# python-microscopy/ch-shrinkwrap

Measured on AMD Instinct MI355X. Metric: vertex-updates/s (force+CG step) + achieved HBM GB/s, 1M pts/200k verts, higher is better.
Workload: dtype f32; 1 GPU; BASELINE configs[2]: two-lobe vesicle (smooth union of two R=300 nm spheres), 1000000 localizations sigma=10 nm, 198812 vertices / 397620 faces, lams=[10], blocks of 5 iterations, fixed topology; localizations_per_gpu=1000000, vertices_per_gpu=198812, faces_per_gpu=397620, block=5, mode=single, parallelism=single GPU

## Files before the change

### ch_shrinkwrap_amd/build.py

```python
import glob
import os
import subprocess

HERE = os.path.dirname(os.path.abspath(__file__))
LIB = os.path.join(HERE, 'libnanowrap_hip.so')


def _csrc(name):
    return os.path.join(HERE, 'csrc', name)


def _include(name):
    return os.path.join(os.path.dirname(HERE), 'include', name)


HIPCC_FLAGS = ['-O3', '--offload-arch=gfx950', '-fPIC', '-shared', '-ffp-contract=off', '-munsafe-fp-atomics',
               '-fvisibility=hidden', '-Wall', '-Wno-unused-function']
_BASE = ['-O3', '--offload-arch=gfx950', '-fPIC', '-fvisibility=hidden']
_QUERY = _BASE + ['-ffp-contract=off', '-Wall', '-Wno-unused-function']
_BQ_H = [_csrc('nw_bq.h'), _csrc('nw_bq_core.h')]
_BQ = _BQ_H + [_csrc('nw_device.h')]

OBJ_MAIN, OBJ_HOLEPUNCH, OBJ_SURGERY, OBJ_BQ = _csrc('nanowrap.o'), _csrc('nw_holepunch.o'), _csrc('nw_surgery.o'), _csrc('nw_bq.o')
OBJ_ISOSURFACE = _csrc('nw_isosurface.o')
# ... 7 lines not shown
OBJ_PROXIMITY = _csrc('nw_proximity.o')
UNITS = [
    (_csrc('nanowrap.hip'), OBJ_MAIN, sorted(set(glob.glob(_csrc('*.h'))) - set(_BQ_H)) + [_include('nanowrap.h')],
     [f for f in HIPCC_FLAGS if f != '-shared']),
    (_csrc('nw_sort.hip'), _csrc('nw_sort.o'), [], _BASE + ['-Wno-unused-value']),
    (_csrc('nw_remesh_dev.hip'), _csrc('nw_remesh_dev.o'), [_include('nanowrap.h'), _csrc('nw_remesh_plan.h')],
     _BASE + ['-ffp-contract=off', '-Wall', '-Wno-unused-value', '-Wno-unused-function']),
    (_csrc('nw_holepunch.hip'), OBJ_HOLEPUNCH, [_include('nw_holepunch.h')] + _BQ_H, _QUERY),
    (_csrc('nw_surgery.hip'), OBJ_SURGERY, [_include('nw_surgery.h')] + _BQ, _QUERY),
    (_csrc('nw_isosurface.hip'), OBJ_ISOSURFACE, [_include('nw_isosurface.h')] + _BQ_H, _QUERY),
    (_csrc('nw_evaluation.hip'), OBJ_EVALUATION, [_include('nw_evaluation.h'), _csrc('nw_evaluation_core.h')] + _BQ_H, _QUERY),
    (_csrc('nw_simulation.hip'), OBJ_SIMULATION, [_include('nw_simulation.h')] + _BQ_H, _QUERY),
    (_csrc('nw_distance.hip'), OBJ_DISTANCE, [_include('nw_distance.h'), _csrc('nw_distance_core.h')] + _BQ_H, _QUERY),
    (_csrc('nw_neighbours.hip'), OBJ_NEIGHBOURS, [_include('nw_neighbours.h'), _csrc('nw_neighbours_core.h')] + _BQ_H, _QUERY),
    (_csrc('nw_intersections.hip'), OBJ_INTERSECTIONS, [_include('nw_intersections.h'), _csrc('nw_intersections_core.h')] + _BQ_H, _QUERY),
    (_csrc('nw_rays.hip'), OBJ_RAYS, [_include('nw_rays.h'), _csrc('nw_rays_core.h'), _csrc('nw_intersections_core.h')] + _BQ_H, _QUERY),
    (_csrc('nw_volume.hip'), OBJ_VOLUME, [_include('nw_volume.h'), _csrc('nw_volume_core.h'), _csrc('nw_distance_core.h')] + _BQ_H, _QUERY),
    (_csrc('nw_proximity.hip'), OBJ_PROXIMITY, [_include('nw_proximity.h'), _csrc('nw_proximity_core.h'), _csrc('nw_distance_core.h'),
                                                _csrc('nw_intersections_core.h')] + _BQ_H, _QUERY),
    (_csrc('nw_bq.hip'), OBJ_BQ, _BQ, _QUERY),
]
DEPS = sorted(set(d for src, _, extra, _ in UNITS for d in [src] + extra))


def needs_build():
    if not os.path.exists(LIB):
        return True
    t = os.path.getmtime(LIB)
    return any(os.path.getmtime(d) > t for d in DEPS)


def build_hip_library(force=False, verbose=False):
    if not force and not needs_build():
        return LIB
    hipcc = os.environ.get('HIPCC', '/opt/rocm/bin/hipcc')

    def run(cmd):
        if verbose:
            print(' '.join(cmd))
        subprocess.check_call(cmd)

    for src, obj, extra, flags in UNITS:
        if force or not os.path.exists(obj) or os.path.getmtime(obj) < max(os.path.getmtime(d) for d in [src] + extra):
            run([hipcc] + flags + ['-c', '-o', obj, src])
    check_kernel_budgets(verbose=verbose)
    run([hipcc, '--offload-arch=gfx950', '-fPIC', '-shared', '-o', LIB] + [obj for _, obj, _, _ in UNITS])
    return LIB


LLVM_BIN = os.environ.get('NW_LLVM_BIN', '/opt/rocm/lib/llvm/bin')
KERNEL_BUDGETS = {
    'k_nn_wave<false>':               (80, 10 * 1024),
    'k_attract':                      (72, 20 * 1024),
    'k_face_centroids':               (64, 8 * 1024),
    'k_centroid_scatter':             (64, 0),
    'k_scan_final':                   (64, 1024),
    'k_prior_ring':                   (128, 1024),
    'k_prior_directions':             (96, 1024),
    'k_subspace_point_sums':          (128, 1024),
    'k_solve_update':                 (128, 1024),
    'k_hp_empty_faces':               (64, 0),
    'k_hp_pair':                      (64, 8 * 1024),
    'k_hp_prism':                     (176, 0),
    'k_hp_cand_geom':                 (32, 0),
    'k_hp_pair_final':                (16, 0),
    'k_ws_init':                      (16, 0),
    'k_ws_hook':                      (32, 0),
    'k_ws_compress':                  (16, 0),
    'k_ws_number':                    (16, 0),
    'k_ws_stats':                     (64, 0),
    'k_ws_bbox_init':                 (16, 0),
    'k_ws_active':                    (16, 0),
    'k_ws_winding':                   (176, 0),
    'k_ws_lengths':                   (16, 0),
    'k_ws_hist':                      (16, 2048),
    'k_ws_pick':                      (32, 0),
    'k_ws_flag':                      (16, 0),
    'k_iso_count':                    (16, 16 * 1024),
    'k_iso_widen':                    (16, 0),
    'k_iso_smooth':                   (16, 0),
    'k_iso_hist':                     (16, 1024),
    'k_iso_pattern':                  (32, 0),
    'k_iso_compact':                  (16, 0),
    'k_iso_cell_counts':              (16, 0),
    'k_iso_vertices':                 (64, 0),
    'k_iso_quads':                    (32, 0),
    'k_ev_face_setup':                (64, 0),
    'k_ev_node_test':                 (32, 0),
    'k_ev_emit':                      (32, 0),
    'k_ev_nearest':                   (64, 64),
    'k_ev_sum_final':                 (16, 64),
    'k_sim_eval':                     (64, 0),
    'k_sim_normals':                  (72, 0),
    'k_sim_cell_test':                (64, 0),
    'k_sim_cell_split':               (24, 0),
    'k_sim_leaf_test':                (64, 0),
    'k_sim_leaf_emit':                (32, 0),
    'k_sim_project':                  (72, 0),
    'k_sim_loc_error':                (32, 0),
    'k_sim_displace':                 (56, 0),
    'k_sim_background':               (16, 0),
    'k_sim_copy_hist':                (16, 1024),
    'k_sim_copy_equal':               (16, 0),
    'k_sim_copy_keep':                (16, 0),
    'k_sim_copy_emit':                (88, 0),
    'k_md_face_setup':                (64, 0),
    'k_md_rho_reduce':                (24, 64),
# ... 116 lines not shown
```

### ch_shrinkwrap_amd/csrc/nanowrap.hip

```cpp
#include <hip/hip_runtime.h>
#include <cstdio>
#include <cstdlib>
#include <cstring>
#include <cmath>
#include <string>
#include <vector>
#include <algorithm>
#include <chrono>
#include <thread>
#include <atomic>

#include "../../include/nanowrap.h"
#include "nw_kernels.h"
#include "nw_host_copy.h"

int nw_sort_pairs_u32(const unsigned *key_in, unsigned *key_out, const int *val_in, int *val_out, int n, int bits, hipStream_t stream);

static_assert(sizeof(NwIterLogDev) == sizeof(nw_iter_log), "device/host log record mismatch");
static_assert(SC_COUNT <= NW_N_SCALARS, "scalar slots");

#define NW_EXPORT extern "C" __attribute__((visibility("default")))

#include <dlfcn.h>
#include <rccl/rccl.h>
// ... 196 lines not shown
    void *pin_log = nullptr;
    int *pin_flag = nullptr;
    DevBuf<int> done_count;
    int done_expected = 0;
    bool done_launched = false;
    double block_us_ema = 0.0;
    uint64_t block_us_key = 0;
    std::chrono::steady_clock::time_point block_t0;
    int sliced_S = 0, sliced_base = 0;
    int64_t sliced_rows = 0;
    size_t pin_log_bytes = 0;
    void *pin = nullptr;
    size_t pin_bytes = 0;
    void *pin_base = nullptr;
    int pin_sel = 0;
    bool rows_async = false;
    NwHostPool *pool = nullptr;
    std::vector<hipEvent_t> wb_events;
    std::vector<unsigned char> valid_host;

    int profiling = 0;
    std::vector<hipEvent_t> events;
    size_t ev_used = 0;
    double stage_ms[ST_COUNT] = {0};
    int64_t stage_launches[ST_COUNT] = {0};
};

namespace {

int fail(nw_ctx *c, int code, const std::string &msg)
{
    if (c) c->err = msg;
    return code;
}

bool env_on(const char *name) { const char *e = getenv(name); return !(e && atoi(e) == 0); }
int verbose_level() { const char *e = getenv("NW_VERBOSE"); return e ? atoi(e) : 0; }

#define NW_HIP(call)                                                                                         \
    do {                                                                                                     \
        hipError_t e_ = (call);                                                                              \
        if (e_ != hipSuccess)                                                                                \
            return fail(ctx, NW_ERR_HIP, std::string(#call) + ": " + hipGetErrorString(e_));                \
    } while (0)

#define NW_TRY(expr)                                                                                         \
    do {                                                                                                     \
        int r_ = (expr);                                                                                     \
        if (r_ != NW_OK) return r_;                                                                          \
    } while (0)

inline int nblk(int64_t n, int b = NW_BLOCK) { return (int)((n + b - 1) / b); }

int scan_exclusive(nw_ctx *ctx, int *in, int n, int *out, bool zero_input = false, int *tile_sums = nullptr)
{
    const int nb = (n + NW_SCAN_TILE - 1) / NW_SCAN_TILE;
    const bool two_pass = nb <= 4096;
    if (tile_sums && two_pass) {
        hipLaunchKernelGGL(k_scan_final, dim3(nb), dim3(NW_BLOCK), 0, ctx->stream, in, n, tile_sums, out, zero_input ? 1 : 0, 1);
        NW_HIP(hipGetLastError());
        return NW_OK;
    }
    NW_HIP(ctx->scan_tmp.ensure((size_t)nb + 1));
    hipLaunchKernelGGL(k_scan_tile_sums, dim3(nb), dim3(NW_BLOCK), 0, ctx->stream, in, n, ctx->scan_tmp.p);
    if (!two_pass) hipLaunchKernelGGL(k_scan_bsums, dim3(1), dim3(1024), 0, ctx->stream, ctx->scan_tmp.p, nb);
    hipLaunchKernelGGL(k_scan_final, dim3(nb), dim3(NW_BLOCK), 0, ctx->stream, in, n, ctx->scan_tmp.p, out, zero_input ? 1 : 0, two_pass ? 1 : 0);
    NW_HIP(hipGetLastError());
    return NW_OK;
}

float dec_ord(int v)
{
    unsigned u = v >= 0 ? (unsigned)v : (0x80000000u - (unsigned)v);
    float f;
    memcpy(&f, &u, 4);
    return f;
}

int enc_ord(float f)
{
    f = f + 0.0f;
    unsigned u;
    memcpy(&u, &f, 4);
    return f >= 0 ? (int)u : (int)(0x80000000u - u);
}

int minmax3(nw_ctx *ctx, const float *xyz, int64_t n, float lo[3], float hi[3], bool *nonfinite)
{
    NW_HIP(ctx->mm.ensure(8));
    int init[8];
    for (int k = 0; k < 3; ++k) { init[k] = enc_ord(INFINITY); init[3 + k] = enc_ord(-INFINITY); }
    init[6] = 0; init[7] = 0;
    NW_HIP(hipMemcpyAsync(ctx->mm.p, init, sizeof(init), hipMemcpyHostToDevice, ctx->stream));
    const int blocks = (int)std::min<int64_t>(2048, (n + NW_BLOCK - 1) / NW_BLOCK);
    hipLaunchKernelGGL(k_minmax3, dim3(blocks), dim3(NW_BLOCK), 0, ctx->stream, xyz, n, ctx->mm.p, (int *)(ctx->mm.p + 6));
    NW_HIP(hipGetLastError());
    int out[8];
    NW_HIP(hipMemcpyAsync(out, ctx->mm.p, sizeof(out), hipMemcpyDeviceToHost, ctx->stream));
    NW_HIP(hipStreamSynchronize(ctx->stream));
    for (int k = 0; k < 3; ++k) { lo[k] = dec_ord(out[k]); hi[k] = dec_ord(out[3 + k]); }
    if (nonfinite) *nonfinite = out[6] != 0;
    return NW_OK;
}

double desired_cell(const nw_ctx *ctx, double mean_dist, double spacing)
{
    const double ratio = std::max((double)ctx->N, 1.0) / (2.5 * std::max((double)ctx->F, 1.0));
    const double sp = std::max(spacing, 1e-30);
    const double sr = ctx->sigma_eff > 0 ? std::min(std::max(ctx->sigma_eff / sp, 1.0), 16.0) : 4.0;
    double h = 2.9 * sp * std::pow(sr, 0.3) * std::pow(ratio, -0.11);
    const char *e = getenv("NW_CELL_FACTOR");
    if (e && atof(e) > 0) h *= atof(e);
    return std::max(h, 0.5 * mean_dist) * ctx->cell_tune;
}

int ensure_item_done(nw_ctx *ctx)
{
    const size_t want = (size_t)std::max(ctx->nitems, 1) + 256;
    if (!ctx->query_serial.p) {
// ... 993 lines not shown
    if (ctx->profiling) { ctx->ev_used = 0; g_marks.spans.clear(); for (int k = 0; k < ST_COUNT; ++k) { ctx->stage_ms[k] = 0; ctx->stage_launches[k] = 0; } }
    ctx->in_search = true;
    ctx->begin_ops_pending = true;
    return NW_OK;
}

static NwAttractArgs attract_args(const nw_ctx *ctx)
{
    NwAttractArgs a;
    memset(&a, 0, sizeof(a));
    a.F = (int)ctx->F; a.sinv_scalar = ctx->sinv_scalar; a.w_scalar = ctx->w_scalar;
    a.cent_by_face = ctx->cent_tmp.p; a.faces = ctx->faces.p; a.pos = ctx->pos.p;
    a.sinv = ctx->sinv_array ? ctx->sinv.p : nullptr; a.wnorm = ctx->w_array ? ctx->wnorm.p : nullptr; a.dat = ctx->have_data ? ctx->dat.p : nullptr;
    a.mask = ctx->mask.p; a.dist = ctx->dist.p; a.wout = ctx->w.p; a.res = ctx->res.p; a.vidx = ctx->vidx.p; a.vacc = ctx->vacc.p; a.part = ctx->part_a.p;
    a.inv_q = 1.0 / ctx->acc_quantum; a.inv_qw = 1.0 / ctx->w_quantum;
    a.d0 = (ctx->have_boundary && ctx->have_halo_d0) ? ctx->halo_d0.p : nullptr; a.perm = ctx->perm.p;
    return a;
}

static int enqueue_begin_ops(nw_ctx *ctx)
{
    ctx->begin_ops_pending = false;
    const int n = std::max(ctx->search_iters, 1);
    const int flag = (ctx->search_iters <= 0 ? 1 : 0) | ((ctx->search_flags & NW_FLAG_NO_LAST_STEP) ? 2 : 0);
    const int64_t work = std::max<int64_t>(9 * ctx->M, flag & 1 ? 3 * ctx->N : 0);
    const int blocks = (int)std::min<int64_t>(4096, std::max<int64_t>(1, (work + NW_BLOCK - 1) / NW_BLOCK));
    hipLaunchKernelGGL(k_block_begin, dim3(blocks), dim3(NW_BLOCK), 0, ctx->stream, (int)ctx->M, (int64_t)(3 * ctx->N), ctx->pos.p, ctx->meshpos.p, ctx->S.p, ctx->res.p,
                       ctx->vacc.p, (unsigned *)ctx->logs.p, (int)((size_t)n * sizeof(NwIterLogDev) / 4), ctx->state.p, flag, ctx->vacc_dirty ? 1 : 0);
    NW_HIP(hipGetLastError());
    if (!ctx->capturing) ctx->vacc_dirty = false;
    return NW_OK;
}

static bool fuse_fixup() { static const bool on = env_on("NW_FUSE_FIXUP"); return on; }

static bool ring_in_nn() { static const bool on = env_on("NW_RING_IN_NN"); return on; }
static NwRingArgs ring_args(const nw_ctx *ctx)
{
    NwRingArgs r;
    r.M = (int)ctx->M; r.maxdeg = ctx->maxdeg; r.nbr_t = ctx->nbr_t.p; r.meshpos = ctx->meshpos.p; r.nrm = ctx->nrm.p; r.ring4 = ctx->ring4.p; r.ring_a = ctx->ring_a.p;
    return r;
}

static bool attract_in_nn() { static const bool on = env_on("NW_ATTRACT_IN_NN"); return on; }
static int launch_query(nw_ctx *ctx, int it, int parts, bool with_ring, bool with_attract, bool *attract_rode)
{
    if (attract_rode) *attract_rode = false;
    const int64_t F = ctx->F;
    const NwGrid g = ctx->grid;
    if (parts & QP_GRID) {
        StageScope s(ctx, ST_GRID);
        static const bool tile_fuse = env_on("NW_TILE_FUSE");
        int *tiles = tile_fuse ? ctx->ctile.p : nullptr;
        hipLaunchKernelGGL(k_face_centroids, dim3(nblk(F)), dim3(NW_BLOCK), 0, ctx->stream, g, ctx->pos.p, ctx->faces.p, (int)F,
                           ctx->cent_tmp.p, ctx->fcell.p, ctx->frank.p, ctx->ccount.p, tiles, ctx->ambig_count.p, ctx->state.p, it, ctx->query_serial.p);
        NW_TRY(scan_exclusive(ctx, ctx->ccount.p, g.ncell, ctx->cstart.p, true, tiles));
        hipLaunchKernelGGL(k_centroid_scatter, dim3(nblk(F)), dim3(NW_BLOCK), 0, ctx->stream, (int)F, ctx->cent_tmp.p, ctx->fcell.p, ctx->frank.p, ctx->cstart.p,
                           ctx->cent.p, ctx->state.p, it, ctx->ctile.p, (g.ncell + NW_SCAN_TILE - 1) / NW_SCAN_TILE);
    }
    if (parts & QP_NN) {
        StageScope s(ctx, ST_NN, it == ctx->search_iters - 1);
        static const int nn_map = getenv("NW_NN_MAP") ? (atoi(getenv("NW_NN_MAP")) == 0 ? 0 : (atoi(getenv("NW_NN_MAP")) == 1 ? 2 : 4)) : 4;
        static const bool no_outliers = getenv("NW_NO_OUTLIERS") != nullptr;
        static const bool item_times = getenv("NW_ITEM_TIMES") != nullptr;
        static const float outl_f = getenv("NW_OUTL_F") ? (float)atof(getenv("NW_OUTL_F")) : 6.25f;
        static const int outl_max = getenv("NW_OUTL_MAX") ? atoi(getenv("NW_OUTL_MAX")) : NW_OUTLIERS;
        static const int tb = getenv("NW_NN_BLOCK") ? std::max(64, std::min(256, atoi(getenv("NW_NN_BLOCK")) & ~63)) : 128;
        const int wpb = tb / 64, nb = (ctx->nitems + wpb - 1) / wpb;
        const int nbp = nn_map == 4 ? (8 * NW_XCD_RUN) * ((nb + 8 * NW_XCD_RUN - 1) / (8 * NW_XCD_RUN)) : 8 * ((nb + 7) / 8);
        NwRingArgs R = ring_args(ctx);
        const bool ring_here = with_ring && ring_in_nn();
        if (!ring_here) R.M = 0;
        const int nbq = nbp;
        const int nbr = ring_here ? 8 * (int)(((ctx->M + tb - 1) / tb + 7) / 8) : 0;
        const bool attract_here = with_attract && attract_in_nn() && fuse_fixup() && ctx->item_done.p != nullptr && tb <= 128 && !ctx->handoff_off;
        const int nbt = nbq + nbr + (attract_here ? nbq : 0);
        const NwAttractArgs AA = attract_args(ctx);
        int *done_p = attract_here ? ctx->item_done.p : nullptr;
        if (attract_here) { ctx->attract_rows = nbq; if (attract_rode) *attract_rode = true; }
        if (ctx->nn_stats.p) {
            hipLaunchKernelGGL(k_nn_wave<true>, dim3(nbt), dim3(tb), 0, ctx->stream, g, ctx->items.p, ctx->nitems, ctx->pts.p, ctx->cstart.p, ctx->cent.p,
                           ctx->cent_tmp.p, (int)F, ctx->face.p, (ctx->face_warm ? 1 : 0) | nn_map | (fuse_fixup() ? 8 : 0) | (no_outliers ? 16 : 0) | (item_times ? 64 : 0), ctx->ambig_list.p, ctx->ambig_count.p,
                           ctx->state.p, it, ctx->nn_stats.p, (ctx->items_by_cost && !item_times) ? nullptr : ctx->item_cost.p, ctx->face_sorted ? ctx->face_orig.p : nullptr, outl_f, outl_max, R, nbq, nbr, AA, done_p, ctx->query_serial.p);
        } else {
            hipLaunchKernelGGL(k_nn_wave<false>, dim3(nbt), dim3(tb), 0, ctx->stream, g, ctx->items.p, ctx->nitems, ctx->pts.p, ctx->cstart.p, ctx->cent.p,
                           ctx->cent_tmp.p, (int)F, ctx->face.p, (ctx->face_warm ? 1 : 0) | nn_map | (fuse_fixup() ? 8 : 0) | (no_outliers ? 16 : 0) | (item_times ? 64 : 0), ctx->ambig_list.p, ctx->ambig_count.p,
                           ctx->state.p, it, ctx->nn_stats.p, (ctx->items_by_cost && !item_times) ? nullptr : ctx->item_cost.p, ctx->face_sorted ? ctx->face_orig.p : nullptr, outl_f, outl_max, R, nbq, nbr, AA, done_p, ctx->query_serial.p);
        }
        if (ctx->face_warm && !ctx->items_by_cost) ctx->item_cost_valid = true;
        ctx->face_warm = true;
    }
    if ((parts & QP_FIXUP) && !fuse_fixup()) {
        StageScope s(ctx, ST_FIXUP);
        static const int fb = getenv("NW_FIXUP_BLOCKS") ? std::max(64, atoi(getenv("NW_FIXUP_BLOCKS"))) : 2048;
        hipLaunchKernelGGL(k_nn_fixup, dim3(fb), dim3(NW_BLOCK), 0, ctx->stream, g, ctx->ambig_list.p, ctx->ambig_count.p, ctx->pts.p, ctx->cstart.p, ctx->cent.p,
                           ctx->cent_tmp.p, ctx->face.p, ctx->state.p, it, ctx->face_sorted ? ctx->face_orig.p : nullptr);
    }
    NW_HIP(hipGetLastError());
    return NW_OK;
}

static int iter_attract_parts(nw_ctx *ctx, int parts)
{
    if (ctx->begin_ops_pending) NW_TRY(enqueue_begin_ops(ctx));
    const int it = ctx->search_done;
    const int64_t N = ctx->N;
    const bool attract_rides = (parts & QP_NN) && (parts & QP_ATTRACT) && attract_in_nn() && fuse_fixup() && ctx->item_done.p != nullptr && ctx->face_warm && !ctx->handoff_off;
    bool rode = false;
    if (parts & (QP_GRID | QP_NN | QP_FIXUP)) NW_TRY(launch_query(ctx, it, parts & (QP_GRID | QP_NN | QP_FIXUP), true, attract_rides, &rode));
// ... 893 lines not shown
        if (hipStreamSynchronize(ctx->stream) != hipSuccess) { rc = NW_ERR_HIP; break; }
    } while (0);
    if (rc != NW_OK) return fail(ctx, rc, "nw_curvature: HIP failure");
    return NW_OK;
}

static int debug_items(nw_ctx *ctx, int32_t *out_items, uint32_t *out_cost, int cap, int *n)
{
    if (!ctx || !n) return NW_ERR_BADARG;
    *n = ctx->nitems;
    const int m = std::min(cap, ctx->nitems);
    NW_HIP(hipStreamSynchronize(ctx->stream));
    if (out_items && m > 0) NW_HIP(hipMemcpy(out_items, ctx->items.p, (size_t)m * sizeof(NwItem), hipMemcpyDeviceToHost));
    if (out_cost && m > 0) NW_HIP(hipMemcpy(out_cost, ctx->item_cost.p, (size_t)m * sizeof(unsigned), hipMemcpyDeviceToHost));
    if (out_cost && m > 0 && getenv("NW_ITEM_TIMES")) NW_HIP(hipMemcpy(out_cost + cap, ctx->item_cost.p + ctx->nitems, (size_t)m * sizeof(unsigned), hipMemcpyDeviceToHost));
    return NW_OK;
}

static int debug_nn_stats(nw_ctx *ctx, int64_t *out)
{
    if (!ctx || !out) return NW_ERR_BADARG;
    if (!ctx->nn_stats.p) {
        NW_HIP(ctx->nn_stats.ensure((size_t)NWS_COUNT * NWS_COPIES));
        NW_HIP(hipMemset(ctx->nn_stats.p, 0, (size_t)NWS_COUNT * NWS_COPIES * sizeof(unsigned long long)));
        for (int k = 0; k <= NWS_COUNT; ++k) out[k] = 0;
        return NW_OK;
    }
    std::vector<unsigned long long> h((size_t)NWS_COUNT * NWS_COPIES);
    NW_HIP(hipStreamSynchronize(ctx->stream));
    NW_HIP(hipMemcpy(h.data(), ctx->nn_stats.p, h.size() * sizeof(unsigned long long), hipMemcpyDeviceToHost));
    NW_HIP(hipMemset(ctx->nn_stats.p, 0, h.size() * sizeof(unsigned long long)));
    for (int k = 0; k < NWS_COUNT; ++k) {
        unsigned long long v = 0;
        for (int c = 0; c < NWS_COPIES; ++c) v = (k == NWS_T_WAVE_MAX) ? std::max(v, h[(size_t)c * NWS_COUNT + k]) : v + h[(size_t)c * NWS_COUNT + k];
        out[k] = (int64_t)v;
    }
    out[NWS_COUNT] = ctx->nitems;
    return NW_OK;
}

NW_EXPORT int nw_debug(nw_ctx *ctx, int what, void *a, void *b, int cap, int *n)
{
    if (what == 0) return debug_nn_stats(ctx, (int64_t *)a);
    if (what == 1) return debug_items(ctx, (int32_t *)a, (uint32_t *)b, cap, n);
    if (what == 2 && ctx && a) {
        ((int64_t *)a)[0] = ctx->n_staged_copy_outs; ((int64_t *)a)[1] = ctx->n_write_backs;
        return NW_OK;
    }
    if (what == 3 && ctx) {
        if (ctx->in_search) return fail(ctx, NW_ERR_BADARG, "nw_debug(3) inside a search");
        ctx->handoff_off = cap != 0;
        return NW_OK;
    }
    return NW_ERR_BADARG;
}

NW_EXPORT int nw_accumulator_quantum(nw_ctx *ctx, double *q)
{
    if (!ctx || !q) return NW_ERR_BADARG;
    if (*q != 0 && ctx->in_search && ctx->search_done > 0) return fail(ctx, NW_ERR_BADARG, "nw_accumulator_quantum: cannot change the quantum between the iterations of a search");
    if (*q > 0 && std::isfinite(*q)) {
        int e = 0;
        const double m = std::frexp(*q, &e);
        ctx->quantum_override = std::ldexp(1.0, m == 0.5 ? e - 1 : e);
        if (ctx->in_search) ctx->acc_quantum = ctx->quantum_override;
    } else if (*q < 0) {
        ctx->quantum_override = 0.0;
        if (ctx->in_search) ctx->acc_quantum = ctx->local_quantum;
    }
    if (!ctx->in_search && ctx->have_points && ctx->have_mesh) {
        NW_HIP(hipSetDevice(ctx->device));
        NW_TRY(alloc_work(ctx));
        NW_TRY(ensure_grid(ctx));
        ctx->local_quantum = std::ldexp(1.0, (int)std::ceil(std::log2(std::max(ctx->scene_ext * ctx->w_bound, 1e-300))) - 36);
    }
    *q = ctx->local_quantum;
    return NW_OK;
}

NW_EXPORT int nw_set_profiling(nw_ctx *ctx, int enable)
{
    if (!ctx) return NW_ERR_BADARG;
    if (enable == 3) return fail(ctx, NW_ERR_BADARG, "nw_set_profiling: level 3 (sampled, two half-block graphs) was removed; use 4");
    ctx->profiling = enable < 0 ? 0 : (enable > 4 ? 4 : enable);
    return NW_OK;
}

NW_EXPORT int nw_stage_ms(nw_ctx *ctx, int stage, double *ms, int64_t *launches)
{
    if (!ctx || stage < 0 || stage >= ST_COUNT) return NW_ERR_BADARG;
    if (ms) *ms = ctx->stage_ms[stage];
    if (launches) *launches = ctx->stage_launches[stage];
    return NW_OK;
}
```

### ch_shrinkwrap_amd/csrc/nw_kernels.h

```cpp
#pragma once
#include "nw_device.h"

enum {
    SC_RES2 = 0,
    SC_C0 = 1,
    SC_SUMD = 2,
    SC_NPTS = 3,
    SC_HC = 4,
    SC_GC = 10,
    SC_STATUS = 13,
    SC_NPOINT = 14,
    SC_SS = 14,
    SC_SP = 20,
    SC_PP64 = 23,
    SC_PP32 = 24,
    SC_T = 25,
    SC_MAXD = 28,
    SC_COUNT = 29
};

#define NW_SPARTS 32

struct NwDevState {
    int stop_at;
    int ntests;
    float tests[3];
    int status;
    int nn_max_ring;
    int iter_base;
    int grid_escape;
};

__global__ void k_set_iter_base(NwDevState *st, int base) { st->iter_base = base; st->grid_escape = 0; }

#define NW_SCAN_TILE 2048

__global__ __launch_bounds__(NW_BLOCK) void k_scan_tile_sums(const int *__restrict__ in, int n, int *__restrict__ bsum)
{
    __shared__ int s_w[4];
    const int base = blockIdx.x * NW_SCAN_TILE + threadIdx.x * 8;
    int s = 0;
#pragma unroll
    for (int k = 0; k < 8; ++k) s += (base + k < n) ? in[base + k] : 0;
#pragma unroll
    for (int off = 32; off > 0; off >>= 1) s += __shfl_xor(s, off, 64);
    if ((threadIdx.x & 63) == 0) s_w[threadIdx.x >> 6] = s;
    __syncthreads();
    if (threadIdx.x == 0) bsum[blockIdx.x] = s_w[0] + s_w[1] + s_w[2] + s_w[3];
}

__global__ __launch_bounds__(1024) void k_scan_bsums(int *__restrict__ bsum, int nb)
{
    __shared__ int s_w[16];
    __shared__ int s_carry;
    if (threadIdx.x == 0) s_carry = 0;
    __syncthreads();
    const int lane = threadIdx.x & 63, wv = threadIdx.x >> 6;
    for (int base = 0; base < nb; base += 1024) {
        const int i = base + threadIdx.x;
        const int v = i < nb ? bsum[i] : 0;
        int inc = nw_wave_incl_scan(v, lane);
        if (lane == 63) s_w[wv] = inc;
        __syncthreads();
        int woff = 0;
        for (int w = 0; w < wv; ++w) woff += s_w[w];
        const int carry = s_carry;
        if (i < nb) bsum[i] = carry + woff + inc - v;
        __syncthreads();
        if (threadIdx.x == 1023) s_carry = carry + woff + inc;
        __syncthreads();
    }
}

__global__ __launch_bounds__(NW_BLOCK) void k_scan_final(int *__restrict__ in, int n, const int *__restrict__ bsum, int *__restrict__ out, int zero_input, int bsum_is_raw)
{
    __shared__ int s_w[4];
    __shared__ int s_pre[4];
    const int lane = threadIdx.x & 63, wv = threadIdx.x >> 6;
    const int base = blockIdx.x * NW_SCAN_TILE + threadIdx.x * 8;
    int v[8];
    int s = 0;
#pragma unroll
    for (int k = 0; k < 8; ++k) { v[k] = (base + k < n) ? in[base + k] : 0; s += v[k]; }
    if (zero_input)
#pragma unroll
        for (int k = 0; k < 8; ++k) if (base + k < n) in[base + k] = 0;
    const int inc = nw_wave_incl_scan(s, lane);
    if (lane == 63) s_w[wv] = inc;
    int pre = 0;
    if (bsum_is_raw) {
        for (int b = threadIdx.x; b < (int)blockIdx.x; b += NW_BLOCK) pre += bsum[b];
#pragma unroll
        for (int o = 32; o > 0; o >>= 1) pre += __shfl_xor(pre, o, 64);
        if (lane == 0) s_pre[wv] = pre;
    }
    __syncthreads();
    int off = (bsum_is_raw ? (s_pre[0] + s_pre[1]) + (s_pre[2] + s_pre[3]) : bsum[blockIdx.x]) + inc - s;
    for (int w = 0; w < wv; ++w) off += s_w[w];
#pragma unroll
    for (int k = 0; k < 8; ++k) {
        if (base + k < n) out[base + k] = off;
        off += v[k];
        if (base + k == n - 1) out[n] = off;
    }
}

__global__ __launch_bounds__(NW_BLOCK) void k_minmax3(const float *__restrict__ xyz, int64_t n, float *__restrict__ mm , int *__restrict__ nonfinite)
{
    __shared__ float s_lo[3][4], s_hi[3][4];
    float lo[3] = {INFINITY, INFINITY, INFINITY}, hi[3] = {-INFINITY, -INFINITY, -INFINITY};
    int bad = 0;
    for (int64_t i = blockIdx.x * (int64_t)blockDim.x + threadIdx.x; i < n; i += (int64_t)gridDim.x * blockDim.x)
        for (int k = 0; k < 3; ++k) {
            const float v = xyz[3 * i + k];
            if (!isfinite(v)) bad = 1;
            lo[k] = fminf(lo[k], v);
            hi[k] = fmaxf(hi[k], v);
        }
    for (int k = 0; k < 3; ++k) {
#pragma unroll
        for (int off = 32; off > 0; off >>= 1) {
            lo[k] = fminf(lo[k], __shfl_xor(lo[k], off, 64));
            hi[k] = fmaxf(hi[k], __shfl_xor(hi[k], off, 64));
        }
        if ((threadIdx.x & 63) == 0) { s_lo[k][threadIdx.x >> 6] = lo[k]; s_hi[k][threadIdx.x >> 6] = hi[k]; }
    }
    __syncthreads();
    if (threadIdx.x < 3) {
        const int k = threadIdx.x;
        const float l = fminf(fminf(s_lo[k][0], s_lo[k][1]), fminf(s_lo[k][2], s_lo[k][3]));
        const float h = fmaxf(fmaxf(s_hi[k][0], s_hi[k][1]), fmaxf(s_hi[k][2], s_hi[k][3]));
        atomicMin((int *)&mm[k], l >= 0 ? __float_as_int(l) : (int)(0x80000000u - (unsigned)__float_as_int(l)));
        atomicMax((int *)&mm[3 + k], h >= 0 ? __float_as_int(h) : (int)(0x80000000u - (unsigned)__float_as_int(h)));
    }
    if (bad) atomicOr(nonfinite, 1);
}

__global__ __launch_bounds__(NW_BLOCK) void k_box_moments(const float *__restrict__ xyz, int64_t n, float ox, float oy, float oz, float inv_q,
                                                         float lx, float ly, float lz, float hx, float hy, float hz, unsigned long long *__restrict__ out)
{
    __shared__ unsigned long long s_part[7][4];
    unsigned long long v[7] = {0, 0, 0, 0, 0, 0, 0};
    for (int64_t i = blockIdx.x * (int64_t)blockDim.x + threadIdx.x; i < n; i += (int64_t)gridDim.x * blockDim.x) {
        const float x = xyz[3 * i], y = xyz[3 * i + 1], z = xyz[3 * i + 2];
        if (x < lx || x > hx || y < ly || y > hy || z < lz || z > hz) continue;
        const unsigned long long qx = (unsigned)nw_clampi((int)((x - ox) * inv_q), 0, 65535), qy = (unsigned)nw_clampi((int)((y - oy) * inv_q), 0, 65535),
                                 qz = (unsigned)nw_clampi((int)((z - oz) * inv_q), 0, 65535);
        v[0] += 1; v[1] += qx; v[2] += qy; v[3] += qz; v[4] += qx * qx; v[5] += qy * qy; v[6] += qz * qz;
    }
    for (int k = 0; k < 7; ++k) {
// ... 95 lines not shown
    if (bstart >= 0) start = bstart;
    int cur = start, s = 0;
    while (cur >= 0 && s < NB) {
        const int4 p = P[cur];
        if (next_out) next_out[(int64_t)a * NB + s] = p.y;
        if (face_out) face_out[(int64_t)a * NB + s] = p.w;
        out[s++] = p.x;
        int nxt = -1;
        for (int j = 0; j < n; ++j) if (P[j].x == p.y) { nxt = j; break; }
        if (nxt == start) break;
        cur = nxt;
    }
    for (; s < NB; ++s) {
        out[s] = -1;
        if (next_out) next_out[(int64_t)a * NB + s] = -1;
        if (face_out) face_out[(int64_t)a * NB + s] = -1;
    }
}

__global__ void k_slot_area(int64_t n_slots, const int *__restrict__ slot_face, const int *__restrict__ faces, const float *__restrict__ pos, float *__restrict__ area)
{
    const int64_t i = (int64_t)blockIdx.x * blockDim.x + threadIdx.x;
    if (i >= n_slots) return;
    const int f = slot_face[i];
    if (f < 0) { area[i] = 0.0f; return; }
    const int v0 = faces[3 * f], v1 = faces[3 * f + 1], v2 = faces[3 * f + 2];
    const float a0 = pos[3 * v1] - pos[3 * v0], a1 = pos[3 * v1 + 1] - pos[3 * v0 + 1], a2 = pos[3 * v1 + 2] - pos[3 * v0 + 2];
    const float b0 = pos[3 * v2] - pos[3 * v0], b1 = pos[3 * v2 + 1] - pos[3 * v0 + 1], b2 = pos[3 * v2 + 2] - pos[3 * v0 + 2];
    const float c0 = a1 * b2 - a2 * b1, c1 = a2 * b0 - a0 * b2, c2 = a0 * b1 - a1 * b0;
    const float n = sqrtf((c0 * c0 + c1 * c1) + c2 * c2);
    area[i] = 0.5f * n;
}

__global__ void k_count_mismatch(int64_t n, const int *__restrict__ a, const int *__restrict__ b, int *__restrict__ out)
{
    const int64_t i = (int64_t)blockIdx.x * blockDim.x + threadIdx.x;
    if (i < n && a[i] != b[i]) atomicAdd(out, 1);
}

__global__ void k_nbr_transpose(const int *__restrict__ nbr, int M, int NB, int *__restrict__ nbr_t, int *__restrict__ maxdeg)
{
    const int v = blockIdx.x * blockDim.x + threadIdx.x;
    if (v >= M) return;
    int last = 0;
    for (int s = 0; s < NB; ++s) {
        const int n = nbr[(int64_t)v * NB + s];
        nbr_t[(int64_t)s * M + v] = n;
        if (n >= 0) last = s + 1;
    }
    atomicMax(maxdeg, last);
}


#define NW_FC_HT 512
#define NW_FC_TT 64
__global__ __launch_bounds__(NW_BLOCK) void k_face_centroids(NwGrid g, const float *__restrict__ pos, const int *__restrict__ faces, int F,
                                                            float4 *__restrict__ cent_tmp, int *__restrict__ fcell, int *__restrict__ frank, int *__restrict__ count,
                                                            int *__restrict__ tile_sums, int *__restrict__ ambig_count, NwDevState *__restrict__ st, int it,
                                                            int *__restrict__ query_serial)
{
    if (st->iter_base + it >= st->stop_at) return;
    __shared__ int s_key[NW_FC_HT], s_cnt[NW_FC_HT];
    __shared__ int s_tkey[NW_FC_TT], s_tcnt[NW_FC_TT];
    for (int t = threadIdx.x; t < NW_FC_HT; t += NW_BLOCK) { s_key[t] = -1; s_cnt[t] = 0; }
    if (threadIdx.x < NW_FC_TT) { s_tkey[threadIdx.x] = -1; s_tcnt[threadIdx.x] = 0; }
    __syncthreads();
    const int f = blockIdx.x * blockDim.x + threadIdx.x;
    if (f == 0) { *ambig_count = 0; *query_serial += 1; }
    int slot = 0, local = 0;
    if (f < F) {
        const int a = faces[3 * f], b = faces[3 * f + 1], c = faces[3 * f + 2];
        const float x = ((pos[3 * a] + pos[3 * b]) + pos[3 * c]) / 3.0f;
        const float y = ((pos[3 * a + 1] + pos[3 * b + 1]) + pos[3 * c + 1]) / 3.0f;
        const float z = ((pos[3 * a + 2] + pos[3 * b + 2]) + pos[3 * c + 2]) / 3.0f;
        int ix, iy, iz;
        nw_cell_coords(g, x, y, z, ix, iy, iz);
        const int cell = nw_cell_index(g, ix, iy, iz);
        const float fx = (x - g.ox) * g.inv_h, fy = (y - g.oy) * g.inv_h, fz = (z - g.oz) * g.inv_h;
        if (fx < -1.0f || fy < -1.0f || fz < -1.0f || fx > (float)g.gx + 1.0f || fy > (float)g.gy + 1.0f || fz > (float)g.gz + 1.0f) st->grid_escape = 1;
        cent_tmp[f] = make_float4(x, y, z, __int_as_float(f));
        fcell[f] = cell;
        slot = (int)(((unsigned)cell * 2654435761u) >> 23);
        for (;;) {
            const int old = atomicCAS(&s_key[slot], -1, cell);
            if (old == -1 || old == cell) break;
            slot = (slot + 1) & (NW_FC_HT - 1);
        }
        local = atomicAdd(&s_cnt[slot], 1);
    }
    __syncthreads();
    for (int t = threadIdx.x; t < NW_FC_HT; t += NW_BLOCK) {
        const int key = s_key[t];
        if (key >= 0) {
            const int c = s_cnt[t];
            const int tile = key / NW_SCAN_TILE;
            int ts = tile & (NW_FC_TT - 1), probes = 0;
            for (; tile_sums;) {
                const int old = atomicCAS(&s_tkey[ts], -1, tile);
                if (old == -1 || old == tile) { atomicAdd(&s_tcnt[ts], c); break; }
                if (++probes == NW_FC_TT) { atomicAdd(&tile_sums[tile], c); break; }
                ts = (ts + 1) & (NW_FC_TT - 1);
            }
            s_cnt[t] = atomicAdd(&count[key], c);
        }
    }
    __syncthreads();
    if (tile_sums && threadIdx.x < NW_FC_TT && s_tkey[threadIdx.x] >= 0) atomicAdd(&tile_sums[s_tkey[threadIdx.x]], s_tcnt[threadIdx.x]);
    __syncthreads();
    if (f < F) frank[f] = s_cnt[slot] + local;
}

__global__ __launch_bounds__(NW_BLOCK) void k_centroid_scatter(int F, const float4 *__restrict__ cent_tmp, const int *__restrict__ fcell, const int *__restrict__ frank,
                                                              const int *__restrict__ start, float4 *__restrict__ cent,
                                                              const NwDevState *__restrict__ st, int it, int *__restrict__ tile_sums, int ntiles)
{
    if (st->iter_base + it >= st->stop_at) return;
    const int f = blockIdx.x * blockDim.x + threadIdx.x;
    for (int t = f; t < ntiles; t += (int)(gridDim.x * blockDim.x)) tile_sums[t] = 0;
    if (f >= F) return;
    cent[start[fcell[f]] + frank[f]] = cent_tmp[f];
}

#include "nw_attract.h"
#include "nw_nn.h"

__global__ __launch_bounds__(NW_BLOCK) void k_nn_fixup(NwGrid g, const int *__restrict__ ambig_list, const int *__restrict__ ambig_count, const float4 *__restrict__ pts,
                                                      const int *__restrict__ cstart, const float4 *__restrict__ cent, const float4 *__restrict__ cent_by_face,
                                                      int *__restrict__ face_out, const NwDevState *__restrict__ st, int it, const int *__restrict__ face_orig)
{
    if (st->iter_base + it >= st->stop_at) return;
    const int na = *ambig_count;
    const int lane = threadIdx.x & 63;
    const int wave = (blockIdx.x * blockDim.x + threadIdx.x) >> 6, nwaves = (gridDim.x * blockDim.x) >> 6;
    for (int a = wave; a < na; a += nwaves) {
        const int gi = ambig_list[a];
        const float4 P = pts[gi];
        const int bf = nw_fixup_point(g, P.x, P.y, P.z, cent_by_face[face_out[gi]], cstart, cent, lane, face_orig);
        if (lane == 0) face_out[gi] = bf;
    }
}

#define NW_HT 512
#define NW_HT_BITS 9
#define NW_ATTRACT_PPT 1
#define NW_HT_PROBES 48

__global__ __launch_bounds__(NW_BLOCK) void k_attract(int N, const float4 *__restrict__ pts, const int *__restrict__ face, const NwAttractArgs A,
                                                     NwDevState *__restrict__ st, int it)
{
    if (st->iter_base + it >= st->stop_at) return;
    __shared__ int s_key[NW_HT];
    __shared__ unsigned long long s_val[NW_HT * 4];
    for (int t = threadIdx.x; t < NW_HT; t += NW_BLOCK) s_key[t] = -1;
    for (int t = threadIdx.x; t < NW_HT * 4; t += NW_BLOCK) s_val[t] = 0ull;
    __syncthreads();
    const int blk = nw_xcd_remap(blockIdx.x, (N + NW_BLOCK * NW_ATTRACT_PPT - 1) / (NW_BLOCK * NW_ATTRACT_PPT));
    double red[4] = {0.0, 0.0, 0.0, 0.0};
    float dmax = 0.0f;
#pragma unroll 1
    for (int pp = 0; pp < NW_ATTRACT_PPT; ++pp) {
        const int i = blk < 0 ? N : (blk * NW_ATTRACT_PPT + pp) * (int)blockDim.x + (int)threadIdx.x;
        const int f_raw = i < N ? face[i] : 0;
// ... 984 lines not shown
```

Baseline: 765.9 million vertex-updates/s.

## Process two faces per thread in centroid binning and prefetch before stop test

k_face_centroids now handles two faces per thread with a larger shared hash table, loads face indices and vertex positions before reading the stop flag so the global loads overlap, and issues the global count atomic before the tile-sum probing. k_scan_final likewise hoists its input and block-sum loads ahead of a new early-exit stop test. A debug query path for dumping grid state is also added. The aim is to cut latency and launch width in the grid-build stage, at the cost of more registers and LDS per workgroup and inline-asm tricks to keep the loads from being sunk.

```diff
diff --git a/ch_shrinkwrap_amd/build.py b/ch_shrinkwrap_amd/build.py
--- a/ch_shrinkwrap_amd/build.py
+++ b/ch_shrinkwrap_amd/build.py
@@ -83,7 +83,7 @@
 KERNEL_BUDGETS = {
     'k_nn_wave<false>':               (80, 10 * 1024),
     'k_attract':                      (72, 20 * 1024),
-    'k_face_centroids':               (64, 8 * 1024),
+    'k_face_centroids':               (64, 10 * 1024),
     'k_centroid_scatter':             (64, 0),
     'k_scan_final':                   (64, 1024),
     'k_prior_ring':                   (128, 1024),
diff --git a/ch_shrinkwrap_amd/csrc/nanowrap.hip b/ch_shrinkwrap_amd/csrc/nanowrap.hip
--- a/ch_shrinkwrap_amd/csrc/nanowrap.hip
+++ b/ch_shrinkwrap_amd/csrc/nanowrap.hip
@@ -272,19 +272,20 @@
 
 inline int nblk(int64_t n, int b = NW_BLOCK) { return (int)((n + b - 1) / b); }
 
-int scan_exclusive(nw_ctx *ctx, int *in, int n, int *out, bool zero_input = false, int *tile_sums = nullptr)
-{
+int scan_exclusive(nw_ctx *ctx, int *in, int n, int *out, bool zero_input = false, int *tile_sums = nullptr, int it = -1)
+{
+    const NwDevState *st = it >= 0 ? ctx->state.p : nullptr;
     const int nb = (n + NW_SCAN_TILE - 1) / NW_SCAN_TILE;
     const bool two_pass = nb <= 4096;
     if (tile_sums && two_pass) {
-        hipLaunchKernelGGL(k_scan_final, dim3(nb), dim3(NW_BLOCK), 0, ctx->stream, in, n, tile_sums, out, zero_input ? 1 : 0, 1);
+        hipLaunchKernelGGL(k_scan_final, dim3(nb), dim3(NW_BLOCK), 0, ctx->stream, in, n, tile_sums, out, zero_input ? 1 : 0, 1, st, it);
         NW_HIP(hipGetLastError());
         return NW_OK;
     }
     NW_HIP(ctx->scan_tmp.ensure((size_t)nb + 1));
     hipLaunchKernelGGL(k_scan_tile_sums, dim3(nb), dim3(NW_BLOCK), 0, ctx->stream, in, n, ctx->scan_tmp.p);
     if (!two_pass) hipLaunchKernelGGL(k_scan_bsums, dim3(1), dim3(1024), 0, ctx->stream, ctx->scan_tmp.p, nb);
-    hipLaunchKernelGGL(k_scan_final, dim3(nb), dim3(NW_BLOCK), 0, ctx->stream, in, n, ctx->scan_tmp.p, out, zero_input ? 1 : 0, two_pass ? 1 : 0);
+    hipLaunchKernelGGL(k_scan_final, dim3(nb), dim3(NW_BLOCK), 0, ctx->stream, in, n, ctx->scan_tmp.p, out, zero_input ? 1 : 0, two_pass ? 1 : 0, st, it);
     NW_HIP(hipGetLastError());
     return NW_OK;
 }
@@ -1384,9 +1385,9 @@
         StageScope s(ctx, ST_GRID);
         static const bool tile_fuse = env_on("NW_TILE_FUSE");
         int *tiles = tile_fuse ? ctx->ctile.p : nullptr;
-        hipLaunchKernelGGL(k_face_centroids, dim3(nblk(F)), dim3(NW_BLOCK), 0, ctx->stream, g, ctx->pos.p, ctx->faces.p, (int)F,
+        hipLaunchKernelGGL(k_face_centroids, dim3(nblk(F, NW_BLOCK * NW_FC_FPT)), dim3(NW_BLOCK), 0, ctx->stream, g, ctx->pos.p, ctx->faces.p, (int)F,
                            ctx->cent_tmp.p, ctx->fcell.p, ctx->frank.p, ctx->ccount.p, tiles, ctx->ambig_count.p, ctx->state.p, it, ctx->query_serial.p);
-        NW_TRY(scan_exclusive(ctx, ctx->ccount.p, g.ncell, ctx->cstart.p, true, tiles));
+        NW_TRY(scan_exclusive(ctx, ctx->ccount.p, g.ncell, ctx->cstart.p, true, tiles, it));
         hipLaunchKernelGGL(k_centroid_scatter, dim3(nblk(F)), dim3(NW_BLOCK), 0, ctx->stream, (int)F, ctx->cent_tmp.p, ctx->fcell.p, ctx->frank.p, ctx->cstart.p,
                            ctx->cent.p, ctx->state.p, it, ctx->ctile.p, (g.ncell + NW_SCAN_TILE - 1) / NW_SCAN_TILE);
     }
@@ -2386,6 +2387,32 @@
         ctx->handoff_off = cap != 0;
         return NW_OK;
     }
+    if (what == 4 && ctx && a && ctx->have_mesh) {
+        const NwGrid &g = ctx->grid;
+        const int ntiles = (g.ncell + NW_SCAN_TILE - 1) / NW_SCAN_TILE;
+        NW_HIP(hipStreamSynchronize(ctx->stream));
+        int len = 0;
+        if (cap == 0) {
+            const double v[12] = {g.ox, g.oy, g.oz, g.h, g.inv_h, g.eps, (double)g.gx, (double)g.gy, (double)g.gz, (double)g.ncell, (double)ctx->F, (double)ntiles};
+            memcpy(a, v, sizeof(v));
+            len = 12;
+        } else if (cap == 1) {
+            len = g.ncell + 1;
+            NW_HIP(hipMemcpy(a, ctx->cstart.p, (size_t)len * sizeof(int), hipMemcpyDeviceToHost));
+        } else if (cap == 2) {
+            len = (int)ctx->F;
+            NW_HIP(hipMemcpy(a, ctx->cent.p, (size_t)len * sizeof(float4), hipMemcpyDeviceToHost));
+        } else if (cap == 3) {
+            len = ntiles;
+            NW_HIP(hipMemcpy(a, ctx->ctile.p, (size_t)len * sizeof(int), hipMemcpyDeviceToHost));
+        } else if (cap == 4) {
+            len = (int)ctx->F;
+            if (ctx->face_sorted) NW_HIP(hipMemcpy(a, ctx->face_orig.p, (size_t)len * sizeof(int), hipMemcpyDeviceToHost));
+            else for (int k = 0; k < len; ++k) ((int *)a)[k] = k;
+        } else return NW_ERR_BADARG;
+        if (n) *n = len;
+        return NW_OK;
+    }
     return NW_ERR_BADARG;
 }
 
diff --git a/ch_shrinkwrap_amd/csrc/nw_kernels.h b/ch_shrinkwrap_amd/csrc/nw_kernels.h
--- a/ch_shrinkwrap_amd/csrc/nw_kernels.h
+++ b/ch_shrinkwrap_amd/csrc/nw_kernels.h
@@ -31,6 +31,22 @@
     int grid_escape;
 };
 
+template <class T> __device__ __forceinline__ void nw_keep(const T &v) { asm volatile("" ::"v"(v)); }
+__device__ const int nw_never_stops[8] = {0x7fffffff, 0, 0, 0, 0, 0, 0, 0};
+struct NwStopTest {
+    int stop_at, iter_base;
+    __device__ __forceinline__ explicit NwStopTest(const NwDevState *st)
+    {
+        static_assert(offsetof(NwDevState, stop_at) == 0 && offsetof(NwDevState, iter_base) == 28, "words of the stop test");
+        int zero;
+        asm("v_mov_b32 %0, 0" : "=v"(zero));
+        const int *w = reinterpret_cast<const int *>(st) + zero;
+        stop_at = w[0];
+        iter_base = w[7];
+    }
+    __device__ __forceinline__ bool stopped(int it) const { return __builtin_amdgcn_readfirstlane(iter_base) + it >= __builtin_amdgcn_readfirstlane(stop_at); }
+};
+
 __global__ void k_set_iter_base(NwDevState *st, int base) { st->iter_base = base; st->grid_escape = 0; }
 
 #define NW_SCAN_TILE 2048
@@ -72,16 +88,25 @@
     }
 }
 
-__global__ __launch_bounds__(NW_BLOCK) void k_scan_final(int *__restrict__ in, int n, const int *__restrict__ bsum, int *__restrict__ out, int zero_input, int bsum_is_raw)
+__global__ __launch_bounds__(NW_BLOCK) void k_scan_final(int *__restrict__ in, int n, const int *__restrict__ bsum, int *__restrict__ out, int zero_input, int bsum_is_raw,
+                                                        const NwDevState *__restrict__ st, int it)
 {
     __shared__ int s_w[4];
     __shared__ int s_pre[4];
     const int lane = threadIdx.x & 63, wv = threadIdx.x >> 6;
     const int base = blockIdx.x * NW_SCAN_TILE + threadIdx.x * 8;
+    const NwStopTest stop(st ? st : reinterpret_cast<const NwDevState *>(nw_never_stops));
     int v[8];
+#pragma unroll
+    for (int k = 0; k < 8; ++k) v[k] = in[min(base + k, n - 1)];
+    const int pre0 = bsum[bsum_is_raw ? min((int)threadIdx.x, max((int)blockIdx.x - 1, 0)) : (int)blockIdx.x];
+#pragma unroll
+    for (int k = 0; k < 8; ++k) nw_keep(v[k]);
+    nw_keep(pre0);
+    if (stop.stopped(it)) return;
     int s = 0;
 #pragma unroll
-    for (int k = 0; k < 8; ++k) { v[k] = (base + k < n) ? in[base + k] : 0; s += v[k]; }
+    for (int k = 0; k < 8; ++k) { v[k] = (base + k < n) ? v[k] : 0; s += v[k]; }
     if (zero_input)
 #pragma unroll
         for (int k = 0; k < 8; ++k) if (base + k < n) in[base + k] = 0;
@@ -89,13 +114,14 @@
     if (lane == 63) s_w[wv] = inc;
     int pre = 0;
     if (bsum_is_raw) {
-        for (int b = threadIdx.x; b < (int)blockIdx.x; b += NW_BLOCK) pre += bsum[b];
+        pre = (int)threadIdx.x < (int)blockIdx.x ? pre0 : 0;
+        for (int b = threadIdx.x + NW_BLOCK; b < (int)blockIdx.x; b += NW_BLOCK) pre += bsum[b];
 #pragma unroll
         for (int o = 32; o > 0; o >>= 1) pre += __shfl_xor(pre, o, 64);
         if (lane == 0) s_pre[wv] = pre;
     }
     __syncthreads();
-    int off = (bsum_is_raw ? (s_pre[0] + s_pre[1]) + (s_pre[2] + s_pre[3]) : bsum[blockIdx.x]) + inc - s;
+    int off = (bsum_is_raw ? (s_pre[0] + s_pre[1]) + (s_pre[2] + s_pre[3]) : pre0) + inc - s;
     for (int w = 0; w < wv; ++w) off += s_w[w];
 #pragma unroll
     for (int k = 0; k < 8; ++k) {
@@ -297,48 +323,81 @@
 }
 
 
-#define NW_FC_HT 512
-#define NW_FC_TT 64
+#define NW_FC_FPT 2
+#define NW_FC_HT_BITS 10
+#define NW_FC_HT (1 << NW_FC_HT_BITS)
+#define NW_FC_TT 128
+static_assert(NW_BLOCK * NW_FC_FPT <= NW_FC_HT, "a workgroup must not hold more faces than its cell table has slots");
+static_assert(NW_FC_HT % NW_BLOCK == 0 && NW_FC_TT <= NW_BLOCK, "flush loops");
 __global__ __launch_bounds__(NW_BLOCK) void k_face_centroids(NwGrid g, const float *__restrict__ pos, const int *__restrict__ faces, int F,
                                                             float4 *__restrict__ cent_tmp, int *__restrict__ fcell, int *__restrict__ frank, int *__restrict__ count,
                                                             int *__restrict__ tile_sums, int *__restrict__ ambig_count, NwDevState *__restrict__ st, int it,
                                                             int *__restrict__ query_serial)
 {
-    if (st->iter_base + it >= st->stop_at) return;
     __shared__ int s_key[NW_FC_HT], s_cnt[NW_FC_HT];
     __shared__ int s_tkey[NW_FC_TT], s_tcnt[NW_FC_TT];
+    const NwStopTest stop(st);
+    const int f0 = blockIdx.x * (NW_BLOCK * NW_FC_FPT) + threadIdx.x;
+    nw_i3u vi[NW_FC_FPT];
+#pragma unroll
+    for (int p = 0; p < NW_FC_FPT; ++p) {
+        const int f = f0 + p * NW_BLOCK;
+        vi[p] = *reinterpret_cast<const nw_i3u *>(faces + 3 * (int64_t)(f < F ? f : 0));
+    }
+    nw_f3u pa[NW_FC_FPT], pb[NW_FC_FPT], pc[NW_FC_FPT];
+#pragma unroll
+    for (int p = 0; p < NW_FC_FPT; ++p) {
+        pa[p] = *reinterpret_cast<const nw_f3u *>(pos + 3 * (int64_t)vi[p].x);
+        pb[p] = *reinterpret_cast<const nw_f3u *>(pos + 3 * (int64_t)vi[p].y);
+        pc[p] = *reinterpret_cast<const nw_f3u *>(pos + 3 * (int64_t)vi[p].z);
+    }
+#pragma unroll
     for (int t = threadIdx.x; t < NW_FC_HT; t += NW_BLOCK) { s_key[t] = -1; s_cnt[t] = 0; }
     if (threadIdx.x < NW_FC_TT) { s_tkey[threadIdx.x] = -1; s_tcnt[threadIdx.x] = 0; }
-    __syncthreads();
-    const int f = blockIdx.x * blockDim.x + threadIdx.x;
-    if (f == 0) { *ambig_count = 0; *query_serial += 1; }
-    int slot = 0, local = 0;
-    if (f < F) {
-        const int a = faces[3 * f], b = faces[3 * f + 1], c = faces[3 * f + 2];
-        const float x = ((pos[3 * a] + pos[3 * b]) + pos[3 * c]) / 3.0f;
-        const float y = ((pos[3 * a + 1] + pos[3 * b + 1]) + pos[3 * c + 1]) / 3.0f;
-        const float z = ((pos[3 * a + 2] + pos[3 * b + 2]) + pos[3 * c + 2]) / 3.0f;
-        int ix, iy, iz;
-        nw_cell_coords(g, x, y, z, ix, iy, iz);
-        const int cell = nw_cell_index(g, ix, iy, iz);
-        const float fx = (x - g.ox) * g.inv_h, fy = (y - g.oy) * g.inv_h, fz = (z - g.oz) * g.inv_h;
-        if (fx < -1.0f || fy < -1.0f || fz < -1.0f || fx > (float)g.gx + 1.0f || fy > (float)g.gy + 1.0f || fz > (float)g.gz + 1.0f) st->grid_escape = 1;
-        cent_tmp[f] = make_float4(x, y, z, __int_as_float(f));
-        fcell[f] = cell;
-        slot = (int)(((unsigned)cell * 2654435761u) >> 23);
-        for (;;) {
-            const int old = atomicCAS(&s_key[slot], -1, cell);
-            if (old == -1 || old == cell) break;
-            slot = (slot + 1) & (NW_FC_HT - 1);
-        }
-        local = atomicAdd(&s_cnt[slot], 1);
-    }
-    __syncthreads();
-    for (int t = threadIdx.x; t < NW_FC_HT; t += NW_BLOCK) {
-        const int key = s_key[t];
-        if (key >= 0) {
+#pragma unroll
+    for (int p = 0; p < NW_FC_FPT; ++p) { nw_keep(pa[p].x); nw_keep(pb[p].x); nw_keep(pc[p].x); }
+    if (stop.stopped(it)) return;
+    __syncthreads();
+    if (f0 == 0) { *ambig_count = 0; *query_serial += 1; }
+    int slot[NW_FC_FPT], local[NW_FC_FPT];
+    bool escaped = false;
+#pragma unroll
+    for (int p = 0; p < NW_FC_FPT; ++p) {
+        const int f = f0 + p * NW_BLOCK;
+        slot[p] = 0; local[p] = 0;
+        if (f < F) {
+            const float x = ((pa[p].x + pb[p].x) + pc[p].x) / 3.0f;
+            const float y = ((pa[p].y + pb[p].y) + pc[p].y) / 3.0f;
+            const float z = ((pa[p].z + pb[p].z) + pc[p].z) / 3.0f;
+            int ix, iy, iz;
+            nw_cell_coords(g, x, y, z, ix, iy, iz);
+            const int cell = nw_cell_index(g, ix, iy, iz);
+            const float fx = (x - g.ox) * g.inv_h, fy = (y - g.oy) * g.inv_h, fz = (z - g.oz) * g.inv_h;
+            if (fx < -1.0f || fy < -1.0f || fz < -1.0f || fx > (float)g.gx + 1.0f || fy > (float)g.gy + 1.0f || fz > (float)g.gz + 1.0f) escaped = true;
+            cent_tmp[f] = make_float4(x, y, z, __int_as_float(f));
+            fcell[f] = cell;
+            int sl = (int)(((unsigned)cell * 2654435761u) >> (32 - NW_FC_HT_BITS));
+            for (;;) {
+                const int old = atomicCAS(&s_key[sl], -1, cell);
+                if (old == -1 || old == cell) break;
+                sl = (sl + 1) & (NW_FC_HT - 1);
+            }
+            slot[p] = sl;
+            local[p] = atomicAdd(&s_cnt[sl], 1);
+        }
+    }
+    if (escaped) st->grid_escape = 1;
+    __syncthreads();
+    int key[NW_FC_HT / NW_BLOCK], base[NW_FC_HT / NW_BLOCK];
+#pragma unroll
+    for (int q = 0; q < NW_FC_HT / NW_BLOCK; ++q) {
+        const int t = threadIdx.x + q * NW_BLOCK;
+        key[q] = s_key[t];
+        base[q] = 0;
+        if (key[q] >= 0) {
             const int c = s_cnt[t];
-            const int tile = key / NW_SCAN_TILE;
+            base[q] = atomicAdd(&count[key[q]], c);
+            const int tile = key[q] / NW_SCAN_TILE;
             int ts = tile & (NW_FC_TT - 1), probes = 0;
             for (; tile_sums;) {
                 const int old = atomicCAS(&s_tkey[ts], -1, tile);
@@ -346,13 +405,19 @@
                 if (++probes == NW_FC_TT) { atomicAdd(&tile_sums[tile], c); break; }
                 ts = (ts + 1) & (NW_FC_TT - 1);
             }
-            s_cnt[t] = atomicAdd(&count[key], c);
         }
     }
     __syncthreads();
     if (tile_sums && threadIdx.x < NW_FC_TT && s_tkey[threadIdx.x] >= 0) atomicAdd(&tile_sums[s_tkey[threadIdx.x]], s_tcnt[threadIdx.x]);
-    __syncthreads();
-    if (f < F) frank[f] = s_cnt[slot] + local;
+#pragma unroll
+    for (int q = 0; q < NW_FC_HT / NW_BLOCK; ++q)
+        if (key[q] >= 0) s_cnt[threadIdx.x + q * NW_BLOCK] = base[q];
+    __syncthreads();
+#pragma unroll
+    for (int p = 0; p < NW_FC_FPT; ++p) {
+        const int f = f0 + p * NW_BLOCK;
+        if (f < F) frank[f] = s_cnt[slot[p]] + local[p];
+    }
 }
 
 __global__ __launch_bounds__(NW_BLOCK) void k_centroid_scatter(int F, const float4 *__restrict__ cent_tmp, const int *__restrict__ fcell, const int *__restrict__ frank,
```

Result: no change. 771.7 million vertex-updates/s, median of 4 (+0.7%).
